# pjmikkol/bwtc

Measured on AMD Instinct MI355X. Metric: MB/s compressed (BWT+encode) on 256 MiB block, higher is better.
Workload: dtype u8/u32/u64 integer

## Files before the change

bwtc_amd/csrc/bwt_engine.hip:

```cpp
#include "bwt_engine.hpp"
#include "radix_sort.hpp"
#include <algorithm>
#include <cmath>
#include <cstdlib>
#include <cstring>
#include <chrono>
#include <climits>
#include <ctime>
#include <sys/prctl.h>

namespace bwtc_hip {

constexpr int kLoadTPB = 256;
constexpr int kLoadTile = kLoadTPB * 16;
constexpr u32 kTextPad = 128;

__global__ __launch_bounds__(kLoadTPB) void k_load_hist(const u8* __restrict__ src,
                                                        u8* __restrict__ T, u32 ncopy,
                                                        u32 padded, int reverse, int aligned,
                                                        u32* __restrict__ freqs) {
  __shared__ __attribute__((aligned(16))) u8 s_src[kLoadTile + 48];
  __shared__ u32 s_hist[256 * 16];
  const u32 tid = threadIdx.x;
  for (u32 i = tid; i < 256 * 16; i += kLoadTPB) s_hist[i] = 0;
// ... 1433 lines not shown
  u32 f = mask ? at + (u32)__builtin_ctzll(mask) : kRunNone;
  for (int o = kWave / 2; o > 0; o >>= 1) f = min(f, (u32)__shfl_xor(f, o, kWave));
  if ((threadIdx.x & (kWave - 1)) == 0) s_min[threadIdx.x / kWave] = f;
  __syncthreads();
  if (threadIdx.x == 0) {
    for (u32 w = 1; w < kRunTPB / kWave; ++w) f = min(f, s_min[w]);
    first[blockIdx.x] = f;
  }
}
__global__ __launch_bounds__(1024) void k_run_carry(const u32* __restrict__ first, u32 tiles, u32 n, u32* __restrict__ behind) {
  __shared__ u32 s_part[1024];
  const u32 per = (tiles + 1023u) / 1024u;
  const u32 lo = min(tiles, threadIdx.x * per), hi = min(tiles, lo + per);
  u32 f = kRunNone;
  for (u32 t = lo; t < hi; ++t) f = min(f, first[t]);
  s_part[threadIdx.x] = f;
  __syncthreads();
  if (threadIdx.x == 0) {
    u32 run = kRunNone;
    for (int i = 1023; i >= 0; --i) { const u32 v = s_part[i]; s_part[i] = run; run = min(run, v); }
  }
  __syncthreads();
  u32 run = s_part[threadIdx.x];
  for (u32 t = hi; t > lo; --t) {
    behind[t - 1u] = run == kRunNone ? n : run;
    run = min(run, first[t - 1u]);
  }
}
template <bool RUN, bool PROPER = false>
__global__ __launch_bounds__(kRunTPB) void k_stretch_lengths(const u8* __restrict__ T, u32 n, u32 p_any, const u32* __restrict__ behind,
                                                              u32* __restrict__ k, u32* __restrict__ longest) {
  __shared__ u64 s_mask[kRunTPB];
  __shared__ u32 s_next[kRunTPB];
  __shared__ u32 s_wave[kRunTPB / kWave];
  const u32 p = RUN ? 1u : p_any;
  const u32 base = blockIdx.x * kRunTile;
  const u32 at = base + threadIdx.x * 64u;
  const u64 mask = stretch_breaks<RUN>(T, at, n, p);
  s_mask[threadIdx.x] = mask;
  __shared__ u64 s_proper[PROPER ? kRunTPB : 1];
  if constexpr (PROPER) s_proper[threadIdx.x] = proper_starts(T, at, n, p);
  const u32 lane = threadIdx.x & (kWave - 1), wave = threadIdx.x / kWave;
  u32 incl = mask ? at + (u32)__builtin_ctzll(mask) : kRunNone;
  for (int o = 1; o < kWave; o <<= 1) {
    const u32 t = __shfl_down(incl, o, kWave);
    if (lane + o < (u32)kWave) incl = min(incl, t);
  }
  if (lane == 0) s_wave[wave] = incl;
  u32 excl = __shfl_down(incl, 1, kWave);
  if (lane == kWave - 1) excl = kRunNone;
  __syncthreads();
  for (u32 w = wave + 1; w < kRunTPB / kWave; ++w) excl = min(excl, s_wave[w]);
  if (excl == kRunNone) excl = behind[blockIdx.x];
  s_next[threadIdx.x] = excl;
  __syncthreads();
  u32 best = 0;
  [[maybe_unused]] u32 best_proper = 0;
  for (u32 j = 0; j < kRunTile / kRunTPB; ++j) {
    const u32 x = base + j * kRunTPB + threadIdx.x;
    const u32 c = j * (kRunTPB / 64u) + wave;
    u32 q, nd;
    if constexpr (RUN) {
      q = x;
      if (q >= n) break;
      const u64 later = lane < 63u ? s_mask[c] >> (lane + 1u) : 0ull;
      nd = later ? q + 1u + (u32)__builtin_ctzll(later) : s_next[c];
    } else {
      if (x < p) continue;
      q = x - p;
      if (q >= n) break;
      const u64 here = s_mask[c] >> lane;
      nd = here ? x + (u32)__builtin_ctzll(here) : s_next[c];
    }
    const u32 kk = min(nd, n) - q;
    if (k) k[q] = kk;
    best = max(best, kk);
    if constexpr (PROPER) { if ((s_proper[c] >> lane) & 1ull) best_proper = max(best_proper, kk); }
  }
  for (int o = kWave / 2; o > 0; o >>= 1) best = max(best, (u32)__shfl_xor(best, o, kWave));
  if (lane == 0 && best) atomicMax(longest, best);
  if constexpr (PROPER) {
    for (int o = kWave / 2; o > 0; o >>= 1) best_proper = max(best_proper, (u32)__shfl_xor(best_proper, o, kWave));
    if (lane == 0 && best_proper) atomicMax(longest + 1, best_proper);
  }
}

constexpr u32 kVoteTPB = 256, kVoteTile = 16384, kVoteBins = kPeriodMax + 1;
constexpr int kSmallPeriod = 802;
constexpr u32 kPeriodMinVotes = 256;
constexpr u64 kPeriodWorth = 8;
template <bool RUNS_OUT>
__global__ __launch_bounds__(kVoteTPB) void k_period_votes(const u64* __restrict__ ks, const u32* __restrict__ vs, u32 m, u64 kmask,
                                                           u32* __restrict__ table, const u32* __restrict__ k1) {
  __shared__ u32 s_bin[kVoteBins];
  for (u32 b = threadIdx.x; b < kVoteBins; b += kVoteTPB) s_bin[b] = 0;
  __syncthreads();
  const u32 base = blockIdx.x * kVoteTile;
  for (u32 j = 0; j < kVoteTile / kVoteTPB; ++j) {
    const u32 i = base + j * kVoteTPB + threadIdx.x;
    if (i + 1u >= m) break;
    if (((ks[i] ^ ks[i + 1u]) & kmask) != 0ull) continue;
    const u32 a = vs[i], b = vs[i + 1u];
    const u32 d = a > b ? a - b : b - a;
    if (d < 2u || d > kPeriodMax) continue;
    if constexpr (RUNS_OUT) { if (k1[min(a, b)] > d) continue; }
    atomicAdd(&s_bin[d], 1u);
  }
  __syncthreads();
  const u32 turn = (blockIdx.x * 67u) % kVoteBins;
  for (u32 b = threadIdx.x; b < kVoteBins; b += kVoteTPB) {
    u32 bb = b + turn;
    if (bb >= kVoteBins) bb -= kVoteBins;
    const u32 c = s_bin[bb];
    if (c) atomicAdd(&table[bb], c);
  }
}
__global__ __launch_bounds__(256) void k_period_probe(const u8* __restrict__ T, u32 n, u32 p, u32 span, u32 windows, u32* flag) {
  const u32 i = blockIdx.x * 256u + threadIdx.x;
  if (i >= windows) return;
  if (*reinterpret_cast<volatile u32*>(flag)) return;
  const u64 x0 = (u64)p + (u64)i * span;
  if (x0 + span > (u64)n) return;
  const u8* a = T + x0;
  const u8* b = a - p;
  for (u32 j = 0; j < span; ++j)
    if (a[j] != b[j]) return;
  atomicOr(flag, 1u);
}
__global__ __launch_bounds__(1024) void k_period_winner(const u32* __restrict__ table, u32* __restrict__ out) {
  __shared__ u64 s_best[1024];
  u64 best = 0;
  for (u32 b = threadIdx.x; b < kVoteBins; b += 1024u) {
    const u64 v = ((u64)table[b] << 32) | (u64)(kVoteBins - b);
    best = v > best ? v : best;
  }
  s_best[threadIdx.x] = best;
  __syncthreads();
  for (u32 o = 512; o > 0; o >>= 1) {
    if (threadIdx.x < o) { const u64 v = s_best[threadIdx.x + o]; if (v > s_best[threadIdx.x]) s_best[threadIdx.x] = v; }
    __syncthreads();
  }
  if (threadIdx.x == 0) {
    const u64 v = s_best[0];
    out[0] = (v >> 32) ? kVoteBins - (u32)v : 0u;
    out[1] = (u32)(v >> 32);
  }
}

__global__ __launch_bounds__(kWinTPB) void k_gather_dense(u64* __restrict__ rec, u32* __restrict__ val,
                                                          const u32* __restrict__ rank,
                                                          const u8* __restrict__ T, u32 m, u32 n, u32 h,
                                                          int b2, int emit, int bin_shift, RunKeys rk) {
  __shared__ u32 s_cnt[256], scr[kWinTPB / kWave + 1];
  __shared__ u32 s_s[kWinTile], s_g[kWinTile];
  u32 blk;
  if (!win_chunk(m, &blk)) return;
  const u32 base = blk * (u32)kWinTile;
  const u32 p0 = base + threadIdx.x;
  u32 s[kWinE], g[kWinE], bin[kWinE], slot[kWinE], okm = 0;
#pragma unroll
  for (int e = 0; e < kWinE; ++e) {
    const u32 p = p0 + e * kWinTPB;
    const bool ok = p < m;
    s[e] = ok ? (u32)(rec[p] >> 32) : 0u;
    g[e] = ok ? val[p] : 0xFFFFFFFFu;
    bin[e] = (s[e] >> bin_shift) & 255u;
// ... 189 lines not shown
  cap = arena_items(max_block_size);
  std::memset(&stats, 0, sizeof stats);
  BWTC_HIP_TRY(hipSetDevice(dev));
  BWTC_HIP_TRY(hipStreamCreateWithFlags(&stream, hipStreamNonBlocking));
  const ArenaPlan a = plan_arena(cap);
  arena_bytes = a.total;
  BWTC_HIP_TRY(hipMalloc(&arena, arena_bytes));
  u8* base = static_cast<u8*>(arena);
  d_T = base + a.off_T;
  d_out = base + a.off_out;
  d_in = base + a.off_in;
  d_SA = reinterpret_cast<u32*>(base + a.off_SA);
  d_rank = reinterpret_cast<u32*>(base + a.off_rank);
  d_R1 = base + a.off_R1;
  d_R2 = base + a.off_R2;
  d_V0 = reinterpret_cast<u32*>(base + a.off_V0);
  d_V1 = reinterpret_cast<u32*>(base + a.off_V1);
  d_G0 = reinterpret_cast<u32*>(base + a.off_G0);
  d_G1 = reinterpret_cast<u32*>(base + a.off_G1);
  d_GRP = reinterpret_cast<u32*>(base + a.off_GRP);
  d_C0 = base + a.off_C0;
  d_C1 = base + a.off_C1;
  d_P0 = base + a.off_P0;
  d_P1 = base + a.off_P1;
  d_W0 = reinterpret_cast<u32*>(base + a.off_W0);
  d_W1 = reinterpret_cast<u32*>(base + a.off_W1);
  d_table = reinterpret_cast<u32*>(base + a.off_table);
  d_partial = reinterpret_cast<u32*>(base + a.off_partial);
  d_aggA = reinterpret_cast<u32*>(base + a.off_aggA);
  d_aggB = reinterpret_cast<u32*>(base + a.off_aggB);
  d_aggC = reinterpret_cast<u32*>(base + a.off_aggC);
  d_agg_part = reinterpret_cast<u32*>(base + a.off_agg_part);
  d_small = reinterpret_cast<u32*>(base + a.off_small);
  d_ent = base + a.off_ent;
  d_comp = base + a.off_comp;
  d_sweep = reinterpret_cast<u32*>(base + a.off_sweep);
  d_parkS = reinterpret_cast<u32*>(base + a.off_parkS);
  d_parkHP = reinterpret_cast<u64*>(base + a.off_parkHP);
  d_hardS = reinterpret_cast<u32*>(base + a.off_hardS);
  d_hardHP = reinterpret_cast<u64*>(base + a.off_hardHP);
  d_hardC = reinterpret_cast<unsigned short*>(base + a.off_hardC);
  d_LP0 = reinterpret_cast<u32*>(base + a.off_LP0);
  d_LH0 = reinterpret_cast<u32*>(base + a.off_LH0);
  d_LH1 = reinterpret_cast<u32*>(base + a.off_LH1);
  d_LC1 = reinterpret_cast<unsigned short*>(base + a.off_LC1);
  d_US = reinterpret_cast<u32*>(base + a.off_US);
  d_UR = reinterpret_cast<u32*>(base + a.off_UR);
  d_pairs = reinterpret_cast<u32*>(base + a.off_pairs);
  d_codes = reinterpret_cast<u32*>(base + a.off_codes);
  d_runK = reinterpret_cast<u32*>(base + a.off_runK);
  d_runF = reinterpret_cast<u32*>(base + a.off_runF);
  d_runB = reinterpret_cast<u32*>(base + a.off_runB);
  d_votes = reinterpret_cast<u32*>(base + a.off_votes);
  use_sweep = env_is("BWTC_HIP_SORT", "sweep");
  wavelet_on_host = env_is("BWTC_HIP_WAVELET", "host");
  device_models = !env_is("BWTC_HIP_MODELS", "host"); models_side_stream = !env_off("BWTC_HIP_MODELS_STREAM");
  int v = 0;
  if (env_int("BWTC_HIP_WAVELET_DEPTH", &v) && v > 0) max_inflight = (unsigned)v;
  dense_route = !env_off("BWTC_HIP_DENSE");
  no_emit = std::getenv("BWTC_HIP_NO_EMIT") != nullptr;
  if (env_int("BWTC_HIP_WINDOW_BITS", &v) && v > 0) window_bits = std::min(24, v);
  digit_planes = !env_off("BWTC_HIP_PLANES"); split_index = !env_off("BWTC_HIP_SPLIT_INDEX");
  if (env_int("BWTC_HIP_GRAMS", &gram_count_override)) gram_keys = !env_off("BWTC_HIP_GRAMS");
  long_keys = !env_off("BWTC_HIP_LONG");
  env_int("BWTC_HIP_LONG_G2", &long_grams_override);
  const bool group_given = env_int("BWTC_HIP_FIN_GROUP", &fin_max_group), window_given = env_int("BWTC_HIP_FIN_WINDOW", &fin_window);
  fin_shape_fixed = group_given || window_given;
  fin_wide_short = !env_off("BWTC_HIP_FIN_WIDE");
  fin_window = fin_window >= 2048 ? 2048 : 1024;
  fin_max_group = fin_max_group >= 1024 ? 1024 : fin_max_group >= 512 ? 512 : 256;
  if (fin_max_group >= fin_window) fin_max_group = fin_window / 2;
  code_keys = !env_is("BWTC_HIP_KEYS", "grams");
  env_int("BWTC_HIP_CODE_BITS", &code_bits, 40, 72);
  finisher = !env_off("BWTC_HIP_FINISHER");
  gm_partition_lines = env_is("BWTC_HIP_GM_PARTITION", "lines");
  wt_segmented = !env_off("BWTC_HIP_SEG_STEPS");
  gram_min_n = kGramMinN;
  if (env_int("BWTC_HIP_GRAM_MIN_N", &v, 64)) gram_min_n = (u32)v;
  if (env_int("BWTC_HIP_LONG_E", &v)) long_items_per_thread = v == 6 ? 6 : 8;
  env_int("BWTC_HIP_FIN_PASSES", &fin_max_passes, 0); env_int("BWTC_HIP_FIN_WORDS", &fin_words, 2, 4);
  long_direct = !env_off("BWTC_HIP_LONG_DIRECT");
  env_int("BWTC_HIP_FIN_ROUNDS", &fin_rounds, 1, 4);
  run_ranks = !env_off("BWTC_HIP_RUNS"); period_ranks = !env_off("BWTC_HIP_PERIODS");
  if (env_int("BWTC_HIP_PERIOD", &v, 0, (int)kPeriodMax)) period_forced = (u32)v;
  mixed_steps = env_is("BWTC_HIP_MIXED", "1");
  local_rounds = !env_off("BWTC_HIP_LOCAL_ROUNDS");
  if (env_int("BWTC_HIP_FIN_FLOOR", &v, 0)) fin_floor = (u32)v;
  text_rounds_fixed = env_int("BWTC_HIP_TEXT_ROUNDS", &text_rounds, 0);
  if (env_int("BWTC_HIP_HUGE_MI", &v) && v > 0) huge_group_elements = (u64)v << 20;
  if (env_is("BWTC_HIP_SCAN", "chained")) {
    scan_chain.cap_tiles = (u32)(cap / kScanTile + 4096);
    BWTC_HIP_TRY(hipMalloc(reinterpret_cast<void**>(&scan_chain.status), ((u64)scan_chain.cap_tiles + 1) * 8));
    BWTC_HIP_TRY(hipMemset(scan_chain.status, 0, ((u64)scan_chain.cap_tiles + 1) * 8));
    scan_chain.ticket = scan_chain.status + scan_chain.cap_tiles;
    scan_chain.err = d_small + 522;
    scan_chain.stream = stream;
    scan_chain.issued = 0;
    scan_chain.epoch = 0;
  }
  BWTC_HIP_TRY(hipHostMalloc(reinterpret_cast<void**>(&h_small), 1024 * 4, hipHostMallocDefault));
  BWTC_HIP_TRY(hipHostMalloc(reinterpret_cast<void**>(&h_stage), cap + 32, hipHostMallocDefault));
  BWTC_HIP_TRY(hipEventCreateWithFlags(&ev_wait, hipEventBlockingSync | hipEventDisableTiming));
  wait_mode = env_is("BWTC_HIP_SYNC", "spin") ? 1 : env_is("BWTC_HIP_SYNC", "block") ? 2 : 0;
  BWTC_HIP_TRY(hipEventCreate(&ev_begin));
  BWTC_HIP_TRY(hipEventCreate(&ev_end));
  for (int i = 0; i < kMaxSortEvents; ++i) BWTC_HIP_TRY(hipEventCreate(&ev_sort[i]));
  return 0;
}

hipError_t BwtEngine::ensure_d2h_stream() {
  if (d2h_stream) return hipSuccess;
  hipError_t rc = hipStreamCreateWithFlags(&d2h_stream, hipStreamNonBlocking);
  if (rc != hipSuccess) return rc;
  rc = hipEventCreateWithFlags(&ev_packed, hipEventDisableTiming);
  if (rc != hipSuccess) return rc;
  rc = hipEventCreateWithFlags(&ev_models, hipEventDisableTiming);
  if (rc != hipSuccess) return rc;
  return hipEventCreateWithFlags(&ev_codes, hipEventBlockingSync | hipEventDisableTiming);
}

hipError_t BwtEngine::codes_wait() {
  if (!codes_in_flight) return hipSuccess;
  codes_in_flight = false;
  return sleepy_wait(ev_codes, kWaitSlots - 1);
}

hipError_t BwtEngine::sleepy_wait(hipEvent_t ev, int slot) {
  using clk = std::chrono::steady_clock;
  static thread_local bool slack_set = false;
  if (!slack_set) { (void)prctl(PR_SET_TIMERSLACK, 1000UL, 0UL, 0UL, 0UL); slack_set = true; }
  const auto t0 = clk::now();
  float& ema = wait_us[slot < 0 ? 0 : slot >= kWaitSlots ? kWaitSlots - 1 : slot];
  double slice = 20.0;
  for (;;) {
    const hipError_t q = hipEventQuery(ev);
    const double el = std::chrono::duration<double, std::micro>(clk::now() - t0).count();
    if (q != hipErrorNotReady) {
      ema = ema > 0.f ? 0.5f * ema + 0.5f * (float)el : (float)el;
      return q;
    }
    const double left = (double)ema - el;
    if (left > 80.0) slice = std::min(200.0, left * 0.25);
    else slice = std::min(200.0, std::max(20.0, slice * 1.25));
    timespec ts;
    ts.tv_sec = 0;
    ts.tv_nsec = (long)(slice * 1e3);
    nanosleep(&ts, nullptr);
  }
}

int BwtEngine::reserve_run_arrays() {
  if (d_run_start[0] && d_run_start[1] && d_run_sym[0] && d_run_sym[1]) return 0;
  bool ok = true;
  for (int b = 0; b < 2; ++b) {
    if (!d_run_start[b]) ok = ok && hipMalloc(reinterpret_cast<void**>(&d_run_start[b]), (cap + 2) * 4) == hipSuccess;
    if (!d_run_sym[b]) ok = ok && hipMalloc(reinterpret_cast<void**>(&d_run_sym[b]), cap + 64) == hipSuccess;
  }
  if (ok) return 0;
  (void)hipGetLastError();
  for (int b = 0; b < 2; ++b) {
    if (d_run_start[b]) (void)hipFree(d_run_start[b]);
    if (d_run_sym[b]) (void)hipFree(d_run_sym[b]);
    d_run_start[b] = nullptr; d_run_sym[b] = nullptr;
  }
  return -2;
}
// ... 778 lines not shown
  hipLaunchKernelGGL(k_raw_to_park, dim3(ceil_div(tied.left, 256)), dim3(256), 0, stream, (const u32*)home.v_free, (const u32*)home.slots_next,
                     (const u32*)d_GRP, tied.left, d_parkS, d_parkHP, blk.fin.parked);
  blk.fin.parked += tied.left;
  *shallow_depth = depth32(tied.h_left);
  if (debug_on()) std::fprintf(stderr, "shallow groups: %u entries still tied at depth %llu join the waiting list\n", tied.left, (unsigned long long)tied.h_left);
  return 0;
}

int BwtEngine::waiting_to_rounds(SortList& L, const FinOutcome& fo, u32 shallow_depth) {
  const FinCounters fc(*this);
  BWTC_HIP_TRY(fc.fetch(kFinWaitDepth, kFinWaitDepth));
  BWTC_HIP_TRY(wait());
  u64 h_pk = std::min<u64>(std::min<u64>(fc[kFinWaitDepth], fo.hard ? fo.hard_depth : 0xFFFFFFFFu), shallow_depth);
  if (blk.fin.local_m) h_pk = std::min<u64>(h_pk, blk.fin.local_depth);
  const u32 total = blk.fin.parked;
  if (debug_on())
    std::fprintf(stderr, "finisher: %u entries (%u of groups too large) go on to the rounds at depth %llu; %u entries of small groups double beside them from depth %u\n",
                 total, fo.hard, (unsigned long long)h_pk, blk.fin.local_m, blk.fin.local_m ? blk.fin.local_depth : 0u);
  if (total) {
    BWTC_HIP_TRY(hipMemcpyAsync(d_V0, d_parkS, (size_t)total * 4, hipMemcpyDeviceToDevice, stream));
    BWTC_HIP_TRY(hipMemcpyAsync(d_R1, d_parkHP, (size_t)total * 8, hipMemcpyDeviceToDevice, stream));
    blk.fin.parked = 0;
    const int rc = dress_list(L, total, d_V0, static_cast<u64*>(d_R1), blk.fin.park_holes);
    if (rc) return rc;
  } else {
    L.res.m = 0; L.res.groups = 0;
    L.home = ListHome::at(d_W0, d_R1, d_V0, d_V1, d_G0, d_G1);
  }
  const u32 listed = total ? L.res.m : 0u;
  const int text_now = (!blk.fin.local_m && ((u64)listed * 16 < (u64)L.n || text_rounds_fixed)) ? text_rounds : 0;
  return run_rounds(L, RoundsRequest{listed, std::max<u64>(1, h_pk), text_now, true, true});
}

int BwtEngine::suffix_sort(u32 n, const u32* hist, bool lone_sentinel, const EmitTarget* em, bool allow_code_keys) {
  n_sort_events = 0;
  stats.rounds = 0; stats.active_sum = 0; stats.sort_pass_items = 0; stats.route = 0; stats.finisher_entries = 0;
  blk = BlockSort{};
  if (n == 0) return 0;

  const KeyPlan plan = plan_keys(hist, n, lone_sentinel, gram_min_n < kGramMinN);
  std::memcpy(h_small + kSmallLut, plan.lut, 256);
  BWTC_HIP_TRY(hipMemcpyAsync(d_small + kSmallLut, h_small + kSmallLut, 256, hipMemcpyHostToDevice, stream));
  const bool implied_idx = !use_sweep && n > 1;
  const InitialSort in{n, hist, lone_sentinel, plan, reinterpret_cast<const u8*>(d_small + kSmallLut),
                       digit_planes && !use_sweep ? d_P0 : nullptr, implied_idx, implied_idx ? nullptr : d_V0};
  RrEmit re{em ? em->out : nullptr, em ? em->out_n : 0u, d_small + kSmallLastChar, d_small + kSmallPidx, d_T, d_C0, nullptr, 0,
            reinterpret_cast<const u8*>(d_small + kSmallInv), d_small + kSmallLf, 0, 0, 0};
  if (em && em->n_lf > 1 && n / em->n_lf >= 1) {
    re.lf_n = em->n_lf; re.lf_x = n / em->n_lf; re.lf_inv = re.lf_x > 1 ? (u32)((1ull << 32) / re.lf_x) : 0u;
  }
  SortList L{n, em != nullptr, ListHome{}, re, RankResult{}, d_C1, true};
  u64 h = (u64)plan.k;

  BWTC_HIP_TRY(hipEventRecord(ev_sort[n_sort_events++], stream));
  int rc = plan.wide ? initial_wide(in, allow_code_keys, L, &h) : initial_keys32(in, L, h);
  if (rc == kCodeTableFull) return suffix_sort(n, hist, lone_sentinel, em, false);
  if (rc) return rc;
  rc = L.res.finish ? finisher_route(L, em->n_lf) : run_rounds(L, RoundsRequest{L.res.m, h, 0, false, true});
  if (rc) return rc;
  BWTC_HIP_TRY(hipGetLastError());
  BWTC_HIP_TRY(take_sticky_error());
  return 0;
}

namespace {
struct PassTimer {
  const bool on = debug_on();
  hipStream_t st;
  hipEvent_t a = nullptr, b = nullptr;
  explicit PassTimer(hipStream_t s) : st(s) {}
  ~PassTimer() { if (a) (void)hipEventDestroy(a); if (b) (void)hipEventDestroy(b); }
  hipError_t start() {
    if (!on) return hipSuccess;
    hipError_t e = hipEventCreate(&a);
    if (e == hipSuccess) e = hipEventCreate(&b);
    return e == hipSuccess ? hipEventRecord(a, st) : e;
  }
  hipError_t stop() { return on ? hipEventRecord(b, st) : hipSuccess; }
  hipError_t ms(float* out) { return hipEventElapsedTime(out, a, b); }
};
}

static constexpr int kSmallStretch = 800;
int BwtEngine::stretch_lengths(u32 n, u32 p, bool store, u32* longest, u32* proper) {
  if (proper) *proper = 0;
  if ((u64)n + p + 2ull * kRunTile > 0xFFFFFFFFull) { *longest = 0; return 0; }
  hipStream_t st = stream;
  const u32 tiles = (u32)(((u64)n + p + kRunTile - 1) / kRunTile);
  u32* k = store ? d_runK : nullptr;
  PassTimer timer(st);
  BWTC_HIP_TRY(hipMemsetAsync(d_small + kSmallStretch, 0, proper ? 8 : 4, st));
  BWTC_HIP_TRY(timer.start());
  if (p == 1 && !proper) {
    hipLaunchKernelGGL(k_stretch_tiles<true>, dim3(tiles), dim3(kRunTPB), 0, st, (const u8*)d_T, n, p, d_runF);
    hipLaunchKernelGGL(k_run_carry, dim3(1), dim3(1024), 0, st, (const u32*)d_runF, tiles, n, d_runB);
    hipLaunchKernelGGL(k_stretch_lengths<true>, dim3(tiles), dim3(kRunTPB), 0, st, (const u8*)d_T, n, p, (const u32*)d_runB, k, d_small + kSmallStretch);
  } else {
    hipLaunchKernelGGL(k_stretch_tiles<false>, dim3(tiles), dim3(kRunTPB), 0, st, (const u8*)d_T, n, p, d_runF);
    hipLaunchKernelGGL(k_run_carry, dim3(1), dim3(1024), 0, st, (const u32*)d_runF, tiles, n, d_runB);
    if (proper)
      hipLaunchKernelGGL((k_stretch_lengths<false, true>), dim3(tiles), dim3(kRunTPB), 0, st, (const u8*)d_T, n, p, (const u32*)d_runB, k, d_small + kSmallStretch);
    else
      hipLaunchKernelGGL(k_stretch_lengths<false>, dim3(tiles), dim3(kRunTPB), 0, st, (const u8*)d_T, n, p, (const u32*)d_runB, k, d_small + kSmallStretch);
  }
  BWTC_HIP_TRY(timer.stop());
  BWTC_HIP_TRY(hipMemcpyAsync(h_small + kSmallStretch, d_small + kSmallStretch, proper ? 8 : 4, hipMemcpyDeviceToHost, st));
  BWTC_HIP_TRY(wait());
  if (timer.on) {
    float ms = 0.f;
    BWTC_HIP_TRY(timer.ms(&ms));
    if (p == 1 && store) std::fprintf(stderr, "runs: the run-length pass took %.4f ms for %u suffixes\n", ms, n);
    else std::fprintf(stderr, store ? "periods: the period-length pass took %.4f ms for %u suffixes, period %u\n"
                                    : "periods: a trial pass (no lengths stored) took %.4f ms for %u suffixes, period %u\n", ms, n, p);
  }
  *longest = h_small[kSmallStretch];
  if (proper) *proper = h_small[kSmallStretch + 1];
  if (store) blk.lengths_period = p;
  if (p == 1) blk.run_longest = *longest;
  stats.alg_bytes += (u64)n * ((p == 1 && !proper ? 1 + 1 : 2 + 2) + (store ? 4 : 0)) + (u64)tiles * 16;
  return 0;
}

int BwtEngine::decide_step(u32 n, u32 m, u64 h_first, const u64* ks, const u32* vs, u64 kmask) {
  hipStream_t st = stream;
  if (run_ranks || period_forced == 1) {
    const int rcr = stretch_lengths(n, 1, true, &blk.run_longest);
    if (rcr) return rcr;
    if ((u64)blk.run_longest > h_first) blk.schedule(1, StretchStep::kThisRound);
    if (debug_on())
      std::fprintf(stderr, "runs: longest run %u, the rounds begin at depth %llu: %s\n", blk.run_longest, (unsigned long long)h_first,
                   blk.n_steps ? "run step" : "no run step");
  }
  const bool mixed = mixed_steps && run_ranks && period_forced != 1;
  const bool run_due = blk.n_steps != 0;
  if (!period_ranks || period_forced == 1 || (run_due && !mixed)) return 0;
  const int rcp = find_period(n, ks, vs, m, kmask);
  if (rcp) return rcp;
  const bool voted = period_forced == 0;
  if (blk.period_p >= 2 && voted) {
    const u64 worth = kPeriodWorth * std::max<u64>(h_first, blk.period_p);
    const u32 span = (u32)std::min<u64>((worth - blk.period_p) / 2, 0x40000000ull);
    const u64 windows = (u64)n > blk.period_p + span ? ((u64)n - blk.period_p) / span : 0;
    bool found = false;
    if (windows) {
      BWTC_HIP_TRY(hipMemsetAsync(d_small + kSmallPeriod + 1, 0, 4, st));
      hipLaunchKernelGGL(k_period_probe, dim3((u32)((windows + 255) / 256)), dim3(256), 0, st, (const u8*)d_T, n, blk.period_p, span, depth32(windows), d_small + kSmallPeriod + 1);
      BWTC_HIP_TRY(hipMemcpyAsync(h_small + kSmallPeriod + 1, d_small + kSmallPeriod + 1, 4, hipMemcpyDeviceToHost, st));
      BWTC_HIP_TRY(wait());
      found = h_small[kSmallPeriod + 1] != 0;
      stats.alg_bytes += windows * 2;
    }
    if (!found) {
      if (debug_on()) std::fprintf(stderr, "periods: no window of %u positions of period %u without a break: no period-length pass\n", span, blk.period_p);
      blk.period_p = 0;
    }
  }
  u32* const proper = mixed ? &blk.proper_longest : nullptr;
  const u32& g = mixed ? blk.proper_longest : blk.period_longest;
  const bool store = !run_due;
  if (blk.period_p >= 2) {
    const bool runs_count = !mixed && voted;
    int rcb = (runs_count && !run_ranks) ? stretch_lengths(n, 1, false, &blk.run_longest) : 0;
    if (rcb) return rcb;
    rcb = stretch_lengths(n, blk.period_p, store, &blk.period_longest, proper);
    if (rcb) return rcb;
    if ((runs_count && blk.run_longest >= blk.period_longest) || (voted && (u64)g < kPeriodWorth * std::max<u64>(h_first, blk.period_p)))
      blk.period_p = 0;
  }
  if (blk.period_p >= 2 && voted && (u64)blk.period_p > h_first && (u64)g > blk.period_p) {
    const u32 winner = blk.period_p, longest_voted = blk.period_longest, proper_voted = blk.proper_longest, g_voted = g;
    u32 rest = winner;
    for (u32 q = 2; q <= rest && blk.period_p / q >= 2; ) {
      if (rest % q) { ++q; continue; }
      rest /= q;
      const int rcb = stretch_lengths(n, blk.period_p / q, false, &blk.period_longest, proper);
      if (rcb) return rcb;
      if (g >= g_voted) blk.period_p /= q;
      else while (rest % q == 0) rest /= q;
    }
    blk.period_longest = longest_voted; blk.proper_longest = proper_voted;
    if (blk.period_p != winner) {
      const int rcb = stretch_lengths(n, blk.period_p, store, &blk.period_longest, proper);
      if (rcb) return rcb;
    }
  }
  bool period_step = false;
  if (blk.period_p >= 2 && (u64)blk.period_p <= h_first) {
    if ((u64)g > h_first) {
      if (run_due) {
        const int rcb = stretch_lengths(n, blk.period_p, true, &blk.period_longest, proper);
        if (rcb) return rcb;
      }
      blk.set_step(StretchStep{blk.period_p, StretchStep::kThisRound, 0, run_due});
      period_step = true;
    }
  } else if (blk.period_p >= 2 && g > blk.period_p) {
    blk.schedule(blk.period_p, StretchStep::kWaiting);
    period_step = true;
  }
  if (!period_step) say_no_period_step(*this, h_first);
  return 0;
}

int BwtEngine::find_period(u32 n, const u64* ks, const u32* vs, u32 m, u64 kmask) {
  if (period_forced) { blk.period_p = period_forced; blk.period_votes = 0; return 0; }
  if (m < 2) return 0;
  hipStream_t st = stream;
  PassTimer timer(st);
  const bool timed = timer.on;
  BWTC_HIP_TRY(hipMemsetAsync(d_votes, 0, (size_t)kVoteBins * 4, st));
  BWTC_HIP_TRY(timer.start());
// ... 820 lines not shown
```

bwtc_amd/csrc/bwt_engine.hpp:

```cpp
#pragma once
#include "common.hpp"
#include "bwtc_hip.h"
#include "radix_sort.hpp"
#include "scan.hpp"
#include "wavelet_host.hpp"
#include "wavelet_pipeline.hpp"
#include <sys/mman.h>
#include <condition_variable>
#include <future>
#include <map>
#include <mutex>
#include <thread>
#include <memory>
#include <utility>
#include <cstdlib>
#include <cstring>
#include <functional>
#include <vector>

namespace bwtc { namespace wavelet { namespace gm { struct Task; struct Chunk; } } }

namespace bwtc_hip {

struct RrEmit;
// ... 381 lines not shown
    }
    static ListHome sorted(void* rec_a, void* rec_b, u32* v_a, u32* v_b, u32* slots, u32* slots_next, const void* ks, u32* vs) {
      return at(rec_a, rec_b, v_a, v_b, slots, slots_next).sorted_into(ks, vs);
    }
    void advance(const void* ks, u32* vs) { sorted_into(ks, vs); std::swap(slots, slots_next); }
    void* spare_region(void* a, void* b, void* c) const { return (a != rec_keys && a != rec_free) ? a : (b != rec_keys && b != rec_free) ? b : c; }
  };
  struct RankResult { u32 m, groups; bool finish; u32 text_chars; bool carry; bool ran_run; };
  template <typename K, bool INIT>
  int rank_step(struct SortList& L, const struct RankRequest& rq);
  int next_list(struct SortList& L, u64* ka, u64* kb, u32* va, u32* vb, u32 m_next, int bits, u32 holes, bool drop_holes, u64 key_bytes, bool timed);
  bool dense_route = true;
  bool digit_planes = true;
  u32 pairs_min = 1u << 21;
  int window_bits = 16;
  bool split_index = true;
  bool gram_keys = true;
  int gram_count_override = 0;
  struct GramPlan { int g = 0, G = 0, b = 0; u32 top = 0; };
  int plan_grams(const KeyPlan& plan, u32 n, const u8* d_lut, GramPlan* gp);
  int initial_keys32(const InitialSort& in, SortList& L, u64 h);
  int initial_wide(const InitialSort& in, bool allow_code_keys, SortList& L, u64* h);
  int initial_keys64(const InitialSort& in, const GramPlan& gp, int key_bits, u32 short_len, int split, SortList& L, u64 h);
  int initial_long(const InitialSort& in, const GramPlan& gp, int key_bits, int split, bool coded, SortList& L, u64* h, bool* ranked);
  struct RoundsRequest { u32 m; u64 h0; int text_rounds; bool keep_first, doubling; };
  struct RoundsLeft { u32 left = 0; u64 h_left = 0; };
  int run_rounds(SortList& L, const RoundsRequest& ask, RoundsLeft* out = nullptr);
  int step_due(const SortList& L, u32 m, u64 h_round, u64 h_first, bool text_round, bool* due);
  int finisher_route(SortList& L, u32 n_lf);
  int finisher_shape(u32 n, const RankResult& res);
  int shallow_rounds(SortList& L, const FinOutcome& fo, u32* shallow_depth);
  int waiting_to_rounds(SortList& L, const FinOutcome& fo, u32 shallow_depth);
  hipError_t finisher_begin(u32* S, u32 m, FinWork* w);
  bool no_emit = false;
  bool long_keys = true;
  int long_items_per_thread = 8;
  u32 gram_min_n = 1u << 22;
  bool code_keys = true;
  int code_bits = 72;
  u32* d_pairs = nullptr;
  u32* d_codes = nullptr;
  u32* d_parkS = nullptr;
  u64* d_parkHP = nullptr;
  u32* d_hardS = nullptr;
  u64* d_hardHP = nullptr;
  unsigned short* d_hardC = nullptr;
  u32 fin_floor = 12;
  bool finisher = true;
  int fin_window = 1024;
  int fin_max_group = 256;
  int fin_words = 2;
  bool fin_shape_fixed = false;
  bool fin_wide_short = true;
  bool long_direct = true;
  int fin_rounds = 3;
  int fin_max_passes = 8;
  int text_rounds = 6;
  bool text_rounds_fixed = false;
  void complete_ranks(u32 n, const u32* list_sfx, const u32* list_slot, u32 m, void* pairs_region, void* tmp_region);
  int finisher_passes(FinWork& w, const FinRequest& rq, FinOutcome* fo);
  int local_handover(const FinWork& w, FinOutcome* fo);
  int park_rest(const FinWork& w, const FinRequest& rq, FinOutcome* fo);
  bool local_rounds = true;
  u32* d_LP0 = nullptr; u32* d_LH0 = nullptr; u32* d_LH1 = nullptr; unsigned short* d_LC1 = nullptr;
  u32* d_US = nullptr; u32* d_UR = nullptr;
  struct FinList local_list(int home) const;
  int local_updates();
  int local_pass(u32 n, u64 h_global, struct RrEmit& re);
  int test_finish_pass(FinPassTest& t);
  int test_finisher(bwtc_hip_fin_run& t);
  int test_rank_pass(bwtc_hip_rank_pass& t);
  int test_rank_scan(u32* a, u32* b, u32* c, u32 ntiles, u32* parts_out, u32 parts_cap, u32* counts_out);
  int test_rank_scatter(bool dense, const u32* where, const u32* what, const u64* rec, u32 m, u32 n, int bin_shift, u32* rank);
  int test_round_keys(bwtc_hip_round_keys& t);
  int test_round(bwtc_hip_round& t);
  int dress_list(SortList& L, u32 total, u32* S, u64* HP, u32 holes = 0);
  bool run_ranks = true;
  bool period_ranks = true;
  u32 period_forced = 0;
  bool mixed_steps = false;
  u32* d_runK = nullptr;
  u32* d_runF = nullptr; u32* d_runB = nullptr;
  u32* d_votes = nullptr;
  int stretch_lengths(u32 n, u32 p, bool store, u32* longest, u32* proper = nullptr);
  int find_period(u32 n, const u64* ks, const u32* vs, u32 m, u64 kmask);
  int decide_step(u32 n, u32 m, u64 h_first, const u64* ks, const u32* vs, u64 kmask);
  int long_grams_override = 0;
  void scatter_rank_pairs(u32* pairs, u32* tmp, u32 m, u32 n);
  int load_text(const u8* d_src, u32 ncopy, u32 n, bool reverse, u32* hist_T);
  int test_code_stage(u32 parts, u32 n, const u32* hist, bool lone_sentinel, int kbits, bool split, u8* lut, u32* sigma);
  int transform(const u8* d_src, u8* d_dst, u32 size, bool raw, u32* lf, u32 n_lf, u32* freqs);
};

u64 huffman_compress_bound(u64 size);
int huffman_encode_device(BwtEngine& e, const u8* d_bwt, u32 size, const u32* lf, u32 n_lf,
                          const u32* freqs, u8* d_out, u64 out_cap, u64* out_bytes);

struct WaveletSectionStats {
  std::vector<u32> sections;
  std::vector<u32> run_freqs;
  std::vector<u64> total_runs;
  std::vector<std::vector<std::pair<u32, u32> > > dist;
  std::vector<u32> first_run;
};
int wavelet_section_stats_device(BwtEngine& e, const u8* d_bwt, u32 size, const u32* freqs,
                                 WaveletSectionStats* out, u32* d_run_start = nullptr, u8* d_run_sym = nullptr,
                                 const std::function<void()>* while_waiting = nullptr);

int wavelet_streams_device(BwtEngine& e, const u32* d_run_start, const u8* d_run_sym, u32 n_runs, const std::vector<u32>& first_run,
                           const bwtc::wavelet::StreamPlan& plan, std::vector<u32>* coded_pos,
                           PinnedBytes* codes, bool async_copy = false, const u32** d_packed = nullptr);
int wavelet_models_device(BwtEngine& e, const u32* d_packed, u32 n_coded, const bwtc::wavelet::StreamPlan& plan,
                          const std::vector<u32>& coded_pos, u32 state_in, uint16_t* h_w, u32* h_tail);
int wavelet_models_prepare(BwtEngine& e, const u32* d_packed, u32 n_coded, const bwtc::wavelet::StreamPlan& plan,
                           const std::vector<u32>& coded_pos, GmPass* g, bool read_ends = false, hipStream_t side = nullptr);
int wavelet_models_prepare_tasks(BwtEngine& e, const u32* d_packed, u32 n_coded, const std::vector<bwtc::wavelet::gm::Task>& tasks,
                                 const std::vector<bwtc::wavelet::gm::Chunk>& chunks, GmPass* g, bool read_ends = false,
                                 hipStream_t side = nullptr);
int wavelet_models_run(BwtEngine& e, const GmPass& g, u32 state_in, uint16_t* h_w, u32* h_tail, u32* early_state);

int wavelet_encode_begin(BwtEngine& e, const u8* d_bwt, u32 size, const u32* lf, u32 n_lf,
                         const u32* freqs, unsigned threads, u8* out, u64 out_cap, u64* ticket);
int wavelet_encode_end(BwtEngine& e, u64 ticket, u64* out_bytes);
int wavelet_encode_prepare(BwtEngine& e, const u8* d_bwt, u32 size, const u32* lf, u32 n_lf,
                           const u32* freqs, unsigned threads, u8* out, u64 out_cap, u64* ticket,
                           const std::function<void()>* while_scanning = nullptr);
int wavelet_encode_queue(BwtEngine& e, u64 ticket, u32 state_in, u32* state_out);
int wavelet_join_begun(BwtEngine& e);
void wavelet_pipeline_release(BwtEngine& e);

int inverse_bwt_device(BwtEngine& e, const u8* d_bwt, u8* d_out, u32 size, const u32* lf, u32 n_lf);

}
```

Baseline: 7289.

## Gate the run-length stretch step on estimated rounds saved for unsorted members

Adds a kernel that, after computing run lengths, counts the unsorted list entries whose run exceeds the current depth and sums the doubling rounds the run step would save them. The run step is scheduled only if that saving clears a threshold proportional to the list size (default 32/16 per entry), with an early-exit once the threshold is reached. This avoids an expensive run-ranking step when only a few suffixes benefit, at the cost of an extra pass over the list and a kernel launch. Refusing the step may leave more prefix-doubling rounds for long runs.

```diff
diff --git a/bwtc_amd/csrc/bwt_engine.hip b/bwtc_amd/csrc/bwt_engine.hip
--- a/bwtc_amd/csrc/bwt_engine.hip
+++ b/bwtc_amd/csrc/bwt_engine.hip
@@ -1539,6 +1539,36 @@
   if constexpr (PROPER) {
     for (int o = kWave / 2; o > 0; o >>= 1) best_proper = max(best_proper, (u32)__shfl_xor(best_proper, o, kWave));
     if (lane == 0 && best_proper) atomicMax(longest + 1, best_proper);
+  }
+}
+
+constexpr u32 kWorthTPB = 256, kWorthTile = 16384;
+__global__ __launch_bounds__(kWorthTPB) void k_run_worth(const u32* __restrict__ vs, u32 m, u32 n, const u32* __restrict__ k, u32 h_first,
+                                                         const u32* __restrict__ longest, u64 enough, u32* __restrict__ out) {
+  __shared__ u32 s_members[kWorthTPB / kWave], s_rounds[kWorthTPB / kWave];
+  __shared__ u32 s_done;
+  if (*longest <= h_first) return;
+  unsigned long long* sum = reinterpret_cast<unsigned long long*>(out);
+  if (threadIdx.x == 0) s_done = enough && __hip_atomic_load(sum, __ATOMIC_RELAXED, __HIP_MEMORY_SCOPE_AGENT) >= enough;
+  __syncthreads();
+  if (s_done) return;
+  const u32 base = blockIdx.x * kWorthTile;
+  u32 members = 0, rounds = 0;
+  for (u32 j = 0; j < kWorthTile / kWorthTPB; ++j) {
+    const u32 i = base + j * kWorthTPB + threadIdx.x;
+    if (i >= m) break;
+    const u32 s = vs[i];
+    if (s >= n) continue;
+    const u32 ks = k[s];
+    if (ks > h_first) { ++members; rounds += 31u - (u32)__builtin_clz(ks / h_first); }
+  }
+  for (int o = kWave / 2; o > 0; o >>= 1) { members += (u32)__shfl_xor(members, o, kWave); rounds += (u32)__shfl_xor(rounds, o, kWave); }
+  if ((threadIdx.x & (kWave - 1)) == 0) { s_members[threadIdx.x / kWave] = members; s_rounds[threadIdx.x / kWave] = rounds; }
+  __syncthreads();
+  if (threadIdx.x == 0) {
+    for (u32 w = 1; w < kWorthTPB / kWave; ++w) { members += s_members[w]; rounds += s_rounds[w]; }
+    if (members) atomicAdd(out + 2, members);
+    if (rounds) atomicAdd(sum, (unsigned long long)rounds);
   }
 }
 
@@ -1894,6 +1924,7 @@
   long_direct = !env_off("BWTC_HIP_LONG_DIRECT");
   env_int("BWTC_HIP_FIN_ROUNDS", &fin_rounds, 1, 4);
   run_ranks = !env_off("BWTC_HIP_RUNS"); period_ranks = !env_off("BWTC_HIP_PERIODS");
+  env_int("BWTC_HIP_RUN_WORTH", &run_worth, 0, 1 << 16);
   if (env_int("BWTC_HIP_PERIOD", &v, 0, (int)kPeriodMax)) period_forced = (u32)v;
   mixed_steps = env_is("BWTC_HIP_MIXED", "1");
   local_rounds = !env_off("BWTC_HIP_LOCAL_ROUNDS");
@@ -2838,7 +2869,8 @@
 }
 
 static constexpr int kSmallStretch = 800;
-int BwtEngine::stretch_lengths(u32 n, u32 p, bool store, u32* longest, u32* proper) {
+static constexpr int kSmallWorth = 808;
+int BwtEngine::stretch_lengths(u32 n, u32 p, bool store, u32* longest, u32* proper, RunWorth* worth) {
   if (proper) *proper = 0;
   if ((u64)n + p + 2ull * kRunTile > 0xFFFFFFFFull) { *longest = 0; return 0; }
   hipStream_t st = stream;
@@ -2861,6 +2893,12 @@
   }
   BWTC_HIP_TRY(timer.stop());
   BWTC_HIP_TRY(hipMemcpyAsync(h_small + kSmallStretch, d_small + kSmallStretch, proper ? 8 : 4, hipMemcpyDeviceToHost, st));
+  if (worth && p == 1 && store && worth->m > 0) {
+    BWTC_HIP_TRY(hipMemsetAsync(d_small + kSmallWorth, 0, 12, st));
+    hipLaunchKernelGGL(k_run_worth, dim3(ceil_div(worth->m, kWorthTile)), dim3(kWorthTPB), 0, st, worth->vs, worth->m, n, (const u32*)d_runK,
+                       worth->h_first, (const u32*)(d_small + kSmallStretch), debug_on() ? 0ull : worth->need, d_small + kSmallWorth);
+    BWTC_HIP_TRY(hipMemcpyAsync(h_small + kSmallWorth, d_small + kSmallWorth, 12, hipMemcpyDeviceToHost, st));
+  }
   BWTC_HIP_TRY(wait());
   if (timer.on) {
     float ms = 0.f;
@@ -2873,6 +2911,10 @@
   if (proper) *proper = h_small[kSmallStretch + 1];
   if (store) blk.lengths_period = p;
   if (p == 1) blk.run_longest = *longest;
+  if (worth && p == 1 && store && worth->m > 0) {
+    worth->members = h_small[kSmallWorth + 2]; worth->rounds = (u64)h_small[kSmallWorth] | (u64)h_small[kSmallWorth + 1] << 32;
+    if (*longest > worth->h_first) stats.alg_bytes += (u64)worth->m * (4 + 4);
+  }
   stats.alg_bytes += (u64)n * ((p == 1 && !proper ? 1 + 1 : 2 + 2) + (store ? 4 : 0)) + (u64)tiles * 16;
   return 0;
 }
@@ -2880,9 +2922,17 @@
 int BwtEngine::decide_step(u32 n, u32 m, u64 h_first, const u64* ks, const u32* vs, u64 kmask) {
   hipStream_t st = stream;
   if (run_ranks || period_forced == 1) {
-    const int rcr = stretch_lengths(n, 1, true, &blk.run_longest);
+    const bool gated = run_worth > 0 && period_forced != 1 && m >= kRunWorthMinList && h_first > 0 && h_first <= 0xFFFFFFFFull;
+    RunWorth rw{vs, m, (u32)h_first, ((u64)run_worth * m + 15) / 16};
+    const int rcr = stretch_lengths(n, 1, true, &blk.run_longest, nullptr, gated ? &rw : nullptr);
     if (rcr) return rcr;
-    if ((u64)blk.run_longest > h_first) blk.schedule(1, StretchStep::kThisRound);
+    if ((u64)blk.run_longest > h_first) {
+      const bool worth = !gated || rw.rounds >= rw.need;
+      if (gated && debug_on())
+        std::fprintf(stderr, "runs: %u members above depth %llu, the step saves them %llu rounds, worth it from %llu for %u entries: %s\n",
+                     rw.members, (unsigned long long)h_first, (unsigned long long)rw.rounds, (unsigned long long)rw.need, m, worth ? "kept" : "refused");
+      if (worth) blk.schedule(1, StretchStep::kThisRound);
+    }
     if (debug_on())
       std::fprintf(stderr, "runs: longest run %u, the rounds begin at depth %llu: %s\n", blk.run_longest, (unsigned long long)h_first,
                    blk.n_steps ? "run step" : "no run step");
diff --git a/bwtc_amd/csrc/bwt_engine.hpp b/bwtc_amd/csrc/bwt_engine.hpp
--- a/bwtc_amd/csrc/bwt_engine.hpp
+++ b/bwtc_amd/csrc/bwt_engine.hpp
@@ -487,7 +487,10 @@
   u32* d_runK = nullptr;
   u32* d_runF = nullptr; u32* d_runB = nullptr;
   u32* d_votes = nullptr;
-  int stretch_lengths(u32 n, u32 p, bool store, u32* longest, u32* proper = nullptr);
+  struct RunWorth { const u32* vs; u32 m; u32 h_first; u64 need; u32 members = 0; u64 rounds = 0; };
+  int stretch_lengths(u32 n, u32 p, bool store, u32* longest, u32* proper = nullptr, RunWorth* worth = nullptr);
+  int run_worth = 32;
+  static constexpr u32 kRunWorthMinList = 1u << 20;
   int find_period(u32 n, const u64* ks, const u32* vs, u32 m, u64 kmask);
   int decide_step(u32 n, u32 m, u64 h_first, const u64* ks, const u32* vs, u64 kmask);
   int long_grams_override = 0;
```

Result: slower. 7103 (-2.6%).
